# bzhangGo/zero

Measured on AMD Instinct MI355X. Metric: src+tgt tokens/sec training, Transformer-base d=512 L=6, higher is better.
Workload: dtype bf16; 1 GPU; Transformer-base (d=512, L=6+6, F=2048, h=8, V=32000) training step, B=64 x (src 64 + tgt 64) tokens per GPU, dropout 0.10, label_smooth 0.1, fwd+bwd+allreduce+Adam; model_name=transformer, parallelism=dp1, hip_graph=whole step

## Files before the change

### zero_amd/csrc/zk_attn_dev.h

```cpp
#pragma once
#include "zk_common.h"

typedef __bf16 bf16x8_t __attribute__((ext_vector_type(8)));
typedef float f32x4_t __attribute__((ext_vector_type(4)));

struct AttnArgs {
  const bf16_t* q; const bf16_t* k; const bf16_t* v;
  int ldq, ldk, ldv;
  long bsq, bsk, bsv;
  int kv_group;
  int B, nh, Lq, Lk, d;
  const float* kmask;
  int causal; int q_pos0;
  float scale; float mask_inf;
  const bf16_t* rpr_k; const bf16_t* rpr_v; int max_rel;
  uint32_t thr; float inv_keep; const uint64_t* seed; uint32_t sid;
  int ldmask;
  const int* pos_dev; int pos_flags;
  const float* gq; const float* gd; bf16_t* pb; bf16_t* dsb; int ldg; int nrp;
};

__device__ __forceinline__ void attn_apply_pos(AttnArgs& a) {
  if (a.pos_dev != nullptr) {
    const int t = *a.pos_dev;
// ... 133 lines not shown
}
__device__ __forceinline__ uint32_t half_of4(const uint4& v, int i) {
  const uint32_t w = (i >> 1) == 0 ? v.x : ((i >> 1) == 1 ? v.y : ((i >> 1) == 2 ? v.z : v.w));
  return (i & 1) ? (w >> 16) : (w & 0xffffu);
}
template <bool FRESH = false>
__device__ __forceinline__ void stage_trans(bf16_t* dst, const bf16_t* src, int ld, int row0, int nrows, int tid) {
  if (tid < 128) {
    const int dc = tid & 7, rq = tid >> 3;
    uint4 v[4];
#pragma unroll
    for (int u = 0; u < 4; ++u) {
      const int r = row0 + rq * 4 + u;
      v[u] = make_uint4(0u, 0u, 0u, 0u);
      if (r < nrows) v[u] = zk_ld16<FRESH>(src + (size_t)r * ld + dc * 8);
    }
#pragma unroll
    for (int i = 0; i < 8; ++i) {
      uint2 o;
      o.x = half_of4(v[0], i) | (half_of4(v[1], i) << 16);
      o.y = half_of4(v[2], i) | (half_of4(v[3], i) << 16);
      *reinterpret_cast<uint2*>(dst + (i * 8 + dc) * ALD + rq * 4) = o;
    }
  }
}
__device__ __forceinline__ int chan_of_phys(int q) { return (q & 7) * 8 + (q >> 3); }
struct DirectRegs { uint4 v[2]; };
template <bool FRESH = false>
__device__ __forceinline__ void load_direct(DirectRegs& R, const bf16_t* src, int ld, int row0, int nrows, int tid) {
#pragma unroll
  for (int it = 0; it < 2; ++it) {
    const int t = tid + it * 256;
    const int r = row0 + (t >> 3), c = (t & 7) * 8;
    const uint4 v = zk_ld16<FRESH>(src + (size_t)min(r, nrows - 1) * ld + c);
    R.v[it] = r < nrows ? v : make_uint4(0u, 0u, 0u, 0u);
  }
}
__device__ __forceinline__ void store_direct(bf16_t* dst, const DirectRegs& R, int tid) {
#pragma unroll
  for (int it = 0; it < 2; ++it) {
    const int t = tid + it * 256;
    *reinterpret_cast<uint4*>(dst + (t >> 3) * ALD + (t & 7) * 8) = R.v[it];
  }
}
struct TransRegs { uint4 v[4]; };
template <bool FRESH = false>
__device__ __forceinline__ void load_trans(TransRegs& R, const bf16_t* src, int ld, int row0, int nrows, int t128) {
  const int dc = t128 & 7, rq = t128 >> 3;
#pragma unroll
  for (int u = 0; u < 4; ++u) {
    const int r = row0 + rq * 4 + u;
    const uint4 v = zk_ld16<FRESH>(src + (size_t)min(r, nrows - 1) * ld + dc * 8);
    R.v[u] = r < nrows ? v : make_uint4(0u, 0u, 0u, 0u);
  }
}
__device__ __forceinline__ void store_trans(bf16_t* dst, const TransRegs& R, int t128) {
  const int dc = t128 & 7, rq = t128 >> 3;
#pragma unroll
  for (int i = 0; i < 8; ++i) {
    uint2 o;
    o.x = half_of4(R.v[0], i) | (half_of4(R.v[1], i) << 16);
    o.y = half_of4(R.v[2], i) | (half_of4(R.v[3], i) << 16);
    *reinterpret_cast<uint2*>(dst + (i * 8 + dc) * ALD + rq * 4) = o;
  }
}
__device__ __forceinline__ void store_tile_rows(const bf16_t* tile, bf16_t* dst, size_t ld, int nrows, int tid) {
#pragma unroll
  for (int it = 0; it < 2; ++it) {
    const int t = tid + it * 256;
    const int r = t >> 3, c = (t & 7) * 8;
    if (r < nrows) *reinterpret_cast<uint4*>(dst + (size_t)r * ld + c) = *reinterpret_cast<const uint4*>(tile + r * ALD + c);
  }
}

__device__ __forceinline__ float quad16_max(float v) {
  v = row16_max(v);
  return v;
}
__device__ __forceinline__ float quad16_sum(float v) {
  v = row16_sum(v);
  return v;
}

#define GLD 68
template <int NKT, bool RPR = false>
struct AttnFwdLds {
  static constexpr int BASE = (2 * TQ * ALD + TQ * (NKT * 64 + 8)) * 2;
  static constexpr int BYTES = BASE + (RPR ? 3 * TQ * ALD * 2 + TQ * GLD * 4 : 0);
};
template <int NKT, bool FRESH = false, bool RPR = false, int PRE = 0>
__device__ __forceinline__ void attn_fwd_tile(unsigned char* smem, const AttnArgs& a, bf16_t* __restrict__ out, int ldo,
                                              float* __restrict__ lse, int qt, int h, int b,
                                              const bf16_t* vt_pre = nullptr) {
  static_assert(PRE == 0 || PRE == 1 || (PRE == 3 && NKT == 1), "PRE = 3 is the single-tile self-attention");
  bf16_t* sQ = reinterpret_cast<bf16_t*>(smem);
  bf16_t* sK = sQ + TQ * ALD;
  bf16_t* sP = sK + TQ * ALD;
  constexpr int PLD = NKT * 64 + 8;
  [[maybe_unused]] bf16_t* sRk = reinterpret_cast<bf16_t*>(smem + AttnFwdLds<NKT, false>::BASE);
  [[maybe_unused]] bf16_t* sRvT = sRk + TQ * ALD;
  [[maybe_unused]] bf16_t* sPB = sRvT + TQ * ALD;
  [[maybe_unused]] float* sG = reinterpret_cast<float*>(sPB + TQ * ALD);
  [[maybe_unused]] const int nrel = 2 * a.max_rel + 1;
  const int tid = threadIdx.x, lane = tid & 63, w = tid >> 6;
  const int i0 = qt * TQ;
  const bf16_t* qb = a.q + (size_t)b * a.bsq + h * AD;
  const bf16_t* kb = a.k + (size_t)(b / a.kv_group) * a.bsk + h * AD;
  const bf16_t* vb = a.v + (size_t)(b / a.kv_group) * a.bsv + h * AD;
  const uint64_t seed = a.thr ? *a.seed : 0;

  DirectRegs rQ, rK;
  [[maybe_unused]] DirectRegs rRk;
  TransRegs rVt;
  if (PRE == 0) load_direct<FRESH>(rQ, qb, a.ldq, i0, a.Lq, tid);
  if (PRE != 3) {
    load_direct<FRESH>(rK, kb, a.ldk, 0, a.Lk, tid);
    if (tid < 128) load_trans<FRESH>(rVt, vb, a.ldv, 0, a.Lk, tid);
  }
  if (RPR) {
    load_direct(rRk, a.rpr_k, AD, 0, nrel, tid);
    if (tid >= 128) load_trans(rVt, a.rpr_v, AD, 0, nrel, tid - 128);
  }
  float kbias[NKT * 4];
#pragma unroll
  for (int t = 0; t < NKT * 4; ++t) {
    const int j = t * 16 + (lane & 15);
    kbias[t] = (a.kmask != nullptr && a.kmask[(size_t)(b / a.kv_group) * a.ldmask + min(j, a.Lk - 1)] == 0.f) ? -a.mask_inf : 0.f;
  }
  if (PRE == 0) store_direct(sQ, rQ, tid);
  if (PRE != 3) store_direct(sK, rK, tid);
  if (RPR) {
    store_direct(sRk, rRk, tid);
    if (tid >= 128) store_trans(sRvT, rVt, tid - 128);
  }
  f32x4_t S[NKT * 4];
#pragma unroll
  for (int kt = 0; kt < NKT; ++kt) {
    if (kt > 0) {
      __syncthreads();
      stage_direct<FRESH>(sK, kb, a.ldk, kt * 64, a.Lk, tid);
    }
    __syncthreads();
    const uint4 q0 = frag(sQ, w * 16, 0, lane), q1 = frag(sQ, w * 16, 1, lane);
#pragma unroll
    for (int nt = 0; nt < 4; ++nt) {
      f32x4_t acc = {0.f, 0.f, 0.f, 0.f};
      acc = mfma16(q0, frag(sK, nt * 16, 0, lane), acc);
      acc = mfma16(q1, frag(sK, nt * 16, 1, lane), acc);
      S[kt * 4 + nt] = acc;
    }
  }
  if (RPR) {
    const uint4 q0 = frag(sQ, w * 16, 0, lane), q1 = frag(sQ, w * 16, 1, lane);
#pragma unroll
    for (int nt = 0; nt < 4; ++nt) {
      f32x4_t acc = {0.f, 0.f, 0.f, 0.f};
      acc = mfma16(q0, frag(sRk, nt * 16, 0, lane), acc);
      acc = mfma16(q1, frag(sRk, nt * 16, 1, lane), acc);
#pragma unroll
      for (int r = 0; r < 4; ++r) sG[(w * 16 + (lane >> 4) * 4 + r) * GLD + nt * 16 + (lane & 15)] = acc[r];
    }
    __builtin_amdgcn_s_waitcnt(0xc07f);
    __builtin_amdgcn_wave_barrier();
  }
  const int rbase = i0 + w * 16 + (lane >> 4) * 4;
  float mx[4] = {-INFINITY, -INFINITY, -INFINITY, -INFINITY};
#pragma unroll
// ... 51 lines not shown
      const int il = w * 16 + (lane >> 4) * 4 + r;
      sP[il * PLD + j] = pb16;
      if (RPR) {
        const float pr = (rbase + r < a.Lq && j < a.Lk) ? bf2f(pb16) : 0.f;
        const int ri = rel_index(a.q_pos0 + rbase + r, j, a.max_rel);
        if (ri == 0) tlo[r] += pr;
        else if (ri == 2 * a.max_rel) thi[r] += pr;
        else sPB[il * ALD + ri] = f2bf(pr);
      }
    }
  }
  if (RPR) {
#pragma unroll
    for (int r = 0; r < 4; ++r) {
      const float s0 = row16_sum(tlo[r]), s1 = row16_sum(thi[r]);
      if ((lane & 15) == 0) {
        const int il = w * 16 + (lane >> 4) * 4 + r;
        sPB[il * ALD] = f2bf(s0);
        if (a.max_rel > 0) sPB[il * ALD + 2 * a.max_rel] = f2bf(s1);
      }
    }
  }
  if (a.pb != nullptr) {
    __builtin_amdgcn_s_waitcnt(0xc07f);
    __builtin_amdgcn_wave_barrier();
    rpr_bucket_rows(a, a.pb, b, h, i0, w, lane, [&](int row, int j) { return bf2f(sP[row * PLD + j]); });
  }
  f32x4_t O[4];
#pragma unroll
  for (int nb = 0; nb < 4; ++nb) O[nb] = (f32x4_t){0.f, 0.f, 0.f, 0.f};
#pragma unroll
  for (int kt = 0; kt < NKT; ++kt) {
    __syncthreads();
    if (kt == 0) { if (PRE != 3 && tid < 128) store_trans(sK, rVt, tid); }
    else stage_trans<FRESH>(sK, vb, a.ldv, kt * 64, a.Lk, tid);
    __syncthreads();
    const bf16_t* sVt = PRE == 3 ? vt_pre : sK;
#pragma unroll
    for (int kk = 0; kk < 2; ++kk) {
      const uint4 pa = *reinterpret_cast<const uint4*>(sP + (w * 16 + (lane & 15)) * PLD + kt * 64 + kk * 32 +
                                                       (lane >> 4) * 8);
#pragma unroll
      for (int nb = 0; nb < 4; ++nb) O[nb] = mfma16(pa, frag(sVt, nb * 16, kk, lane), O[nb]);
    }
  }
  if (RPR) {
    __builtin_amdgcn_s_waitcnt(0xc07f);
    __builtin_amdgcn_wave_barrier();
#pragma unroll
    for (int kk = 0; kk < 2; ++kk) {
      const uint4 pa = frag(sPB, w * 16, kk, lane);
#pragma unroll
      for (int nb = 0; nb < 4; ++nb) O[nb] = mfma16(pa, frag(sRvT, nb * 16, kk, lane), O[nb]);
    }
  }
#pragma unroll
  for (int nb = 0; nb < 4; ++nb) {
    const int c = chan_of_phys(nb * 16 + (lane & 15));
#pragma unroll
    for (int r = 0; r < 4; ++r) sQ[(w * 16 + (lane >> 4) * 4 + r) * ALD + c] = f2bf(O[nb][r]);
  }
  __syncthreads();
  store_tile_rows(sQ, out + ((size_t)b * a.Lq + i0) * ldo + h * AD, ldo, a.Lq - i0, tid);
}

#define ATTN_BWD64_LDS_BYTES (7 * TQ * ALD * 2 + TQ * 4)
#define ATTN_BWD64_RPR_LDS_BYTES (ATTN_BWD64_LDS_BYTES + 6 * TQ * ALD * 2 + 2 * TQ * GLD * 4)
struct AttnOProj { const bf16_t* dy; int lddy; const bf16_t* w; int ldw; int n; };
template <bool RPR = false, bool OPROJ = false>
__device__ __forceinline__ void attn_bwd_fused64_tile(unsigned char* smem, const AttnArgs& a, const bf16_t* __restrict__ o, int ldo,
                                                      const bf16_t* __restrict__ dout, int lddo,
                                                      const float* __restrict__ lse,
                                                      bf16_t* __restrict__ dq, int lddq,
                                                      bf16_t* __restrict__ dk, int lddk,
                                                      bf16_t* __restrict__ dv, int lddv, int h, int b,
                                                      float* __restrict__ rpr_part = nullptr,
                                                      const AttnOProj op = AttnOProj()) {
  bf16_t* sQ = reinterpret_cast<bf16_t*>(smem);
  bf16_t* sK = sQ + TQ * ALD;
  bf16_t* sV = sK + TQ * ALD;
  bf16_t* sdO = sV + TQ * ALD;
  bf16_t* sKt = sdO + TQ * ALD;
  bf16_t* sQt = sKt + TQ * ALD;
  bf16_t* sdOt = sQt + TQ * ALD;
  float* sL = reinterpret_cast<float*>(sdOt + TQ * ALD);
  [[maybe_unused]] bf16_t* sRk = reinterpret_cast<bf16_t*>(smem + ATTN_BWD64_LDS_BYTES);
  [[maybe_unused]] bf16_t* sRv = sRk + TQ * ALD;
  [[maybe_unused]] bf16_t* sRkT = sRv + TQ * ALD;
  [[maybe_unused]] bf16_t* sSB = sRkT + TQ * ALD;
  [[maybe_unused]] bf16_t* sSBt = sSB + TQ * ALD;
  [[maybe_unused]] bf16_t* sPBt = sSBt + TQ * ALD;
  [[maybe_unused]] float* sG = reinterpret_cast<float*>(sPBt + TQ * ALD);
  [[maybe_unused]] float* sGd = sG + TQ * GLD;
  const int tid = threadIdx.x, lane = tid & 63, w = tid >> 6;
  const bf16_t* qb = a.q + (size_t)b * a.bsq + h * AD;
  const bf16_t* kb = a.k + (size_t)b * a.bsk + h * AD;
  const bf16_t* vb = a.v + (size_t)b * a.bsv + h * AD;
  (void)o; (void)ldo;
  const bf16_t* dob = dout + (size_t)b * a.Lq * lddo + h * AD;
  const uint64_t seed = a.thr ? *a.seed : 0;

  ZK_AT(0);
  DirectRegs rQ, rdO, rK, rV;
  TransRegs t0, t1;
  load_direct(rQ, qb, a.ldq, 0, a.Lq, tid);
  if (!OPROJ) load_direct(rdO, dob, lddo, 0, a.Lq, tid);
  load_direct(rK, kb, a.ldk, 0, a.Lk, tid);
  load_direct(rV, vb, a.ldv, 0, a.Lk, tid);
  if (tid < 128) {
    load_trans(t0, kb, a.ldk, 0, a.Lk, tid);
  } else {
    load_trans(t0, qb, a.ldq, 0, a.Lq, tid - 128);
    if (!OPROJ) load_trans(t1, dob, lddo, 0, a.Lq, tid - 128);
  }
  [[maybe_unused]] f32x4_t dOa[4];
  [[maybe_unused]] DirectRegs wr[8];
  [[maybe_unused]] uint4 av[16];
  [[maybe_unused]] const bf16_t* wrow = OPROJ ? op.w + (size_t)h * AD * op.ldw : nullptr;
  [[maybe_unused]] const bf16_t* ap =
      OPROJ ? op.dy + ((size_t)b * a.Lq + min(w * 16 + (lane & 15), a.Lq - 1)) * op.lddy + (lane >> 4) * 8 : nullptr;
  auto oproj_issue = [&](int c0) {
    const int nsl = min(4, (op.n - c0) >> 7);
#pragma unroll
    for (int sl = 0; sl < 4; ++sl) {
      if (sl < nsl) {
        load_direct(wr[2 * sl], wrow + c0 + sl * 128, op.ldw, 0, AD, tid);
        load_direct(wr[2 * sl + 1], wrow + c0 + sl * 128 + 64, op.ldw, 0, AD, tid);
#pragma unroll
        for (int u = 0; u < 4; ++u) av[4 * sl + u] = zk_ld16<false>(ap + c0 + sl * 128 + u * 32);
      }
    }
  };
  if (OPROJ) {
#pragma unroll
    for (int nb = 0; nb < 4; ++nb) dOa[nb] = (f32x4_t){0.f, 0.f, 0.f, 0.f};
    oproj_issue(0);
  }
  const int dr = tid >> 2, dpart = tid & 3;
  const int drc = min(dr, a.Lq - 1);
  const float lse_r = lse[((size_t)b * a.nh + h) * a.Lq + drc];
  float kbias4[4];
#pragma unroll
  for (int nt = 0; nt < 4; ++nt) {
    const int j = nt * 16 + (lane & 15);
    kbias4[nt] = (a.kmask != nullptr && a.kmask[(size_t)b * a.ldmask + min(j, a.Lk - 1)] == 0.f) ? -a.mask_inf : 0.f;
  }
  if (OPROJ) {
    ZK_AT(1);
    for (int c0 = 0; c0 < op.n; c0 += 512) {
      const int nsl = min(4, (op.n - c0) >> 7);
      if (c0 > 0) oproj_issue(c0);
      else {
        store_direct(sQ, rQ, tid);
        store_direct(sK, rK, tid);
        store_direct(sV, rV, tid);
      }
#pragma unroll
      for (int sl = 0; sl < 4; ++sl) {
        if (sl < nsl) {
          bf16_t* w0 = sdO + (sl & 1) * 2 * TQ * ALD;
          bf16_t* w1 = w0 + TQ * ALD;
          store_direct(w0, wr[2 * sl], tid);
          store_direct(w1, wr[2 * sl + 1], tid);
          __syncthreads();
#pragma unroll
          for (int nb = 0; nb < 4; ++nb) {
            dOa[nb] = mfma16(av[4 * sl + 0], frag(w0, nb * 16, 0, lane), dOa[nb]);
            dOa[nb] = mfma16(av[4 * sl + 1], frag(w0, nb * 16, 1, lane), dOa[nb]);
            dOa[nb] = mfma16(av[4 * sl + 2], frag(w1, nb * 16, 0, lane), dOa[nb]);
            dOa[nb] = mfma16(av[4 * sl + 3], frag(w1, nb * 16, 1, lane), dOa[nb]);
          }
        }
      }
    }
    ZK_AT(2);
    __syncthreads();
  } else {
    store_direct(sQ, rQ, tid);
    store_direct(sdO, rdO, tid);
    store_direct(sK, rK, tid);
    store_direct(sV, rV, tid);
  }
  if (tid < 128) {
    store_trans(sKt, t0, tid);
  } else {
    store_trans(sQt, t0, tid - 128);
    if (!OPROJ) store_trans(sdOt, t1, tid - 128);
  }
  if (OPROJ) {
    const int r0 = w * 16 + (lane >> 4) * 4;
#pragma unroll
    for (int nb = 0; nb < 4; ++nb) {
      const int c = nb * 16 + (lane & 15);
      uint32_t hv[4];
#pragma unroll
      for (int r = 0; r < 4; ++r) {
        hv[r] = (r0 + r < a.Lq) ? (uint32_t)f2bf(dOa[nb][r]) : 0u;
        sdO[(r0 + r) * ALD + c] = (bf16_t)hv[r];
      }
      *reinterpret_cast<uint2*>(sdOt + ((c & 7) * 8 + (c >> 3)) * ALD + r0) = make_uint2(hv[0] | (hv[1] << 16), hv[2] | (hv[3] << 16));
    }
  }
  if (dpart == 0) sL[dr] = (dr < a.Lq) ? lse_r : 0.f;
  ZK_AT(3);
  if (RPR) {
    const int nrel = 2 * a.max_rel + 1;
    stage_direct(sRk, a.rpr_k, AD, 0, nrel, tid);
    stage_direct(sRv, a.rpr_v, AD, 0, nrel, tid);
    stage_trans(sRkT, a.rpr_k, AD, 0, nrel, tid);
    for (int e = tid; e < 3 * TQ * ALD / 8; e += 256)
      reinterpret_cast<uint4*>(sSB)[e] = make_uint4(0u, 0u, 0u, 0u);
  }
  __syncthreads();
  if (RPR) {
    const uint4 q0 = frag(sQ, w * 16, 0, lane), q1 = frag(sQ, w * 16, 1, lane);
    const uint4 g0 = frag(sdO, w * 16, 0, lane), g1 = frag(sdO, w * 16, 1, lane);
#pragma unroll
    for (int nt = 0; nt < 4; ++nt) {
      f32x4_t ga = {0.f, 0.f, 0.f, 0.f}, gb = {0.f, 0.f, 0.f, 0.f};
      ga = mfma16(q0, frag(sRk, nt * 16, 0, lane), ga);
      ga = mfma16(q1, frag(sRk, nt * 16, 1, lane), ga);
      gb = mfma16(g0, frag(sRv, nt * 16, 0, lane), gb);
      gb = mfma16(g1, frag(sRv, nt * 16, 1, lane), gb);
#pragma unroll
      for (int r = 0; r < 4; ++r) {
        sG[(w * 16 + (lane >> 4) * 4 + r) * GLD + nt * 16 + (lane & 15)] = ga[r];
        sGd[(w * 16 + (lane >> 4) * 4 + r) * GLD + nt * 16 + (lane & 15)] = gb[r];
      }
    }
    __builtin_amdgcn_s_waitcnt(0xc07f);
    __builtin_amdgcn_wave_barrier();
  }
  ZK_AT(4);
  const int rloc = w * 16 + (lane >> 4) * 4;
  float pv[4][4], dsv[4][4];
  {
    float pu[4][4], dpv[4][4], Di[4] = {0.f, 0.f, 0.f, 0.f};
    const uint4 q0 = frag(sQ, w * 16, 0, lane), q1 = frag(sQ, w * 16, 1, lane);
    const uint4 g0 = frag(sdO, w * 16, 0, lane), g1 = frag(sdO, w * 16, 1, lane);
#pragma unroll
    for (int nt = 0; nt < 4; ++nt) {
      f32x4_t sc4 = {0.f, 0.f, 0.f, 0.f}, dp = {0.f, 0.f, 0.f, 0.f};
// ... 9 lines not shown
        const int i = rloc + r;
        const bool live = kvalid && i < a.Lq;
        float raw = sc4[r], dpr = dp[r];
        if (a.gq != nullptr && live) { raw += rpr_gather(a, a.gq, b, h, i, j); dpr += rpr_gather(a, a.gd, b, h, i, j); }
        if (RPR && live) {
          const int ri = rel_index(a.q_pos0 + i, j, a.max_rel);
          raw += sG[i * GLD + ri];
          dpr += sGd[i * GLD + ri];
        }
        float sc = raw * a.scale + kbias;
        if (a.causal && j > a.q_pos0 + i) sc -= a.mask_inf;
        const float p = live ? __expf(sc - sL[i]) : 0.f;
        float ms = 1.f;
        if (a.thr) {
          const uint64_t idx = (((uint64_t)b * a.nh + h) * a.Lq + i) * a.Lk + j;
          ms = zk_drop_scale(seed, a.sid, idx, a.thr, a.inv_keep);
        }
        pv[nt][r] = p * ms;
        pu[nt][r] = p;
        dpv[nt][r] = dpr * ms;
        Di[r] += p * dpr * ms;
      }
    }
#pragma unroll
    for (int r = 0; r < 4; ++r) {
      Di[r] = row16_sum(Di[r]);
    }
#pragma unroll
    for (int nt = 0; nt < 4; ++nt)
#pragma unroll
      for (int r = 0; r < 4; ++r) dsv[nt][r] = pu[nt][r] * (dpv[nt][r] - Di[r]) * a.scale;
  }
  ZK_AT(5);
  __syncthreads();
  ZK_AT(6);
  bf16_t* sdS = sQ;
  bf16_t* sPt = sK;
  bf16_t* sdSt = sV;
#pragma unroll
  for (int nt = 0; nt < 4; ++nt) {
    const int j = nt * 16 + (lane & 15);
    uint2 pp, dd;
    pp.x = (uint32_t)f2bf(pv[nt][0]) | ((uint32_t)f2bf(pv[nt][1]) << 16);
    pp.y = (uint32_t)f2bf(pv[nt][2]) | ((uint32_t)f2bf(pv[nt][3]) << 16);
    dd.x = (uint32_t)f2bf(dsv[nt][0]) | ((uint32_t)f2bf(dsv[nt][1]) << 16);
    dd.y = (uint32_t)f2bf(dsv[nt][2]) | ((uint32_t)f2bf(dsv[nt][3]) << 16);
    *reinterpret_cast<uint2*>(sPt + j * ALD + rloc) = pp;
    *reinterpret_cast<uint2*>(sdSt + j * ALD + rloc) = dd;
#pragma unroll
    for (int r = 0; r < 4; ++r) sdS[(rloc + r) * ALD + j] = f2bf(dsv[nt][r]);
  }
  __syncthreads();
  if (RPR) {
    rpr_bucket_wave(a, 2 * a.max_rel + 1, 0, w, lane, [&](int row, int j) { return bf2f(sdS[row * ALD + j]); },
                    [&](int row, int r, float v) { const bf16_t x = f2bf(v); sSB[row * ALD + r] = x; sSBt[r * ALD + row] = x; });
    rpr_bucket_wave(a, 2 * a.max_rel + 1, 0, w, lane, [&](int row, int j) { return bf2f(sPt[j * ALD + row]); },
                    [&](int row, int r, float v) { sPBt[r * ALD + row] = f2bf(v); });
    __syncthreads();
  }
  if (a.dsb != nullptr) {
    rpr_bucket_rows(a, a.dsb, b, h, 0, w, lane, [&](int row, int j) { return bf2f(sdS[row * ALD + j]); });
    rpr_bucket_rows(a, a.pb, b, h, 0, w, lane, [&](int row, int j) { return bf2f(sPt[j * ALD + row]); });
  }
  ZK_AT(7);
  f32x4_t dQ[4], dK[4], dV[4];
#pragma unroll
  for (int nb = 0; nb < 4; ++nb) {
    dQ[nb] = (f32x4_t){0.f, 0.f, 0.f, 0.f};
    dK[nb] = (f32x4_t){0.f, 0.f, 0.f, 0.f};
    dV[nb] = (f32x4_t){0.f, 0.f, 0.f, 0.f};
  }
#pragma unroll
  for (int kk = 0; kk < 2; ++kk) {
    const uint4 da = frag(sdS, w * 16, kk, lane);
    const uint4 pa = frag(sPt, w * 16, kk, lane);
    const uint4 dt = frag(sdSt, w * 16, kk, lane);
#pragma unroll
    for (int nb = 0; nb < 4; ++nb) {
      dQ[nb] = mfma16(da, frag(sKt, nb * 16, kk, lane), dQ[nb]);
      dV[nb] = mfma16(pa, frag(sdOt, nb * 16, kk, lane), dV[nb]);
      dK[nb] = mfma16(dt, frag(sQt, nb * 16, kk, lane), dK[nb]);
    }
  }
  ZK_AT(8);
  if (RPR) {
    f32x4_t tk[4], tv[4];
#pragma unroll
    for (int nb = 0; nb < 4; ++nb) { tk[nb] = (f32x4_t){0.f, 0.f, 0.f, 0.f}; tv[nb] = (f32x4_t){0.f, 0.f, 0.f, 0.f}; }
#pragma unroll
    for (int kk = 0; kk < 2; ++kk) {
      const uint4 sb = frag(sSB, w * 16, kk, lane);
      const uint4 st = frag(sSBt, w * 16, kk, lane);
      const uint4 pt = frag(sPBt, w * 16, kk, lane);
#pragma unroll
      for (int nb = 0; nb < 4; ++nb) {
        dQ[nb] = mfma16(sb, frag(sRkT, nb * 16, kk, lane), dQ[nb]);
        tk[nb] = mfma16(st, frag(sQt, nb * 16, kk, lane), tk[nb]);
        tv[nb] = mfma16(pt, frag(sdOt, nb * 16, kk, lane), tv[nb]);
      }
    }
    float* pk = rpr_part + ((size_t)b * a.nh + h) * 2 * TQ * AD;
#pragma unroll
    for (int nb = 0; nb < 4; ++nb) {
      const int c = chan_of_phys(nb * 16 + (lane & 15));
#pragma unroll
      for (int r = 0; r < 4; ++r) {
        sG[(rloc + r) * GLD + c] = tk[nb][r];
        sGd[(rloc + r) * GLD + c] = tv[nb][r];
      }
    }
    __builtin_amdgcn_s_waitcnt(0xc07f);
    __builtin_amdgcn_wave_barrier();
    const int nrel = 2 * a.max_rel + 1;
#pragma unroll
    for (int it = 0; it < 4; ++it) {
      const int e = it * 64 + lane, rr = w * 16 + (e >> 4), c4 = (e & 15) * 4;
      if (rr < nrel) {
        *reinterpret_cast<float4*>(pk + rr * AD + c4) = *reinterpret_cast<const float4*>(sG + rr * GLD + c4);
        *reinterpret_cast<float4*>(pk + TQ * AD + rr * AD + c4) = *reinterpret_cast<const float4*>(sGd + rr * GLD + c4);
      }
    }
  }
  __syncthreads();
  bf16_t* oQ = sKt; bf16_t* oK = sQt; bf16_t* oV = sdOt;
#pragma unroll
  for (int nb = 0; nb < 4; ++nb) {
    const int c = chan_of_phys(nb * 16 + (lane & 15));
#pragma unroll
    for (int r = 0; r < 4; ++r) {
      const int i = rloc + r;
      oQ[i * ALD + c] = f2bf(dQ[nb][r]);
      oK[i * ALD + c] = f2bf(dK[nb][r]);
      oV[i * ALD + c] = f2bf(dV[nb][r]);
    }
  }
  __syncthreads();
  ZK_AT(9);
  store_tile_rows(oQ, dq + (size_t)b * a.Lq * lddq + h * AD, lddq, a.Lq, tid);
  store_tile_rows(oK, dk + (size_t)b * a.Lk * lddk + h * AD, lddk, a.Lk, tid);
  store_tile_rows(oV, dv + (size_t)b * a.Lk * lddv + h * AD, lddv, a.Lk, tid);
  ZK_AT(10);
}

#define ATTN_BWD64_RPR2_LDS_BYTES (8 * TQ * ALD * 2 + TQ * 4)
__device__ __forceinline__ void attn_bwd_rpr64_tile(unsigned char* smem, const AttnArgs& a,
                                                    const bf16_t* __restrict__ dout, int lddo,
                                                    const float* __restrict__ lse,
                                                    bf16_t* __restrict__ dq, int lddq,
                                                    bf16_t* __restrict__ dk, int lddk,
                                                    bf16_t* __restrict__ dv, int lddv, int h, int b,
                                                    float* __restrict__ rpr_part) {
  constexpr int TB = TQ * ALD;
  bf16_t* T0 = reinterpret_cast<bf16_t*>(smem);
  bf16_t* T1 = T0 + TB; bf16_t* T2 = T1 + TB; bf16_t* T3 = T2 + TB;
  bf16_t* T4 = T3 + TB; bf16_t* T5 = T4 + TB; bf16_t* T6 = T5 + TB; bf16_t* T7 = T6 + TB;
  float* sG = reinterpret_cast<float*>(T6);
  float* sL = reinterpret_cast<float*>(T7 + TB);
  static_assert(TQ * GLD * 4 <= 2 * TQ * ALD * 2, "G must fit two tiles");
  static_assert(2 * TQ * GLD * 4 <= 4 * TQ * ALD * 2, "the two table partials must fit four tiles");
  const int tid = threadIdx.x, lane = tid & 63, w = tid >> 6;
  const bf16_t* qb = a.q + (size_t)b * a.bsq + h * AD;
  const bf16_t* kb = a.k + (size_t)b * a.bsk + h * AD;
  const bf16_t* vb = a.v + (size_t)b * a.bsv + h * AD;
  const bf16_t* dob = dout + (size_t)b * a.Lq * lddo + h * AD;
  const uint64_t seed = a.thr ? *a.seed : 0;
  const int nrel = 2 * a.max_rel + 1;

  ZK_AT(0);
  DirectRegs rQ, rdO, rK, rV, rRk, rRv;
  TransRegs t0, t1;
  load_direct(rQ, qb, a.ldq, 0, a.Lq, tid);
  load_direct(rdO, dob, lddo, 0, a.Lq, tid);
  load_direct(rK, kb, a.ldk, 0, a.Lk, tid);
  load_direct(rV, vb, a.ldv, 0, a.Lk, tid);
  load_direct(rRk, a.rpr_k, AD, 0, nrel, tid);
  load_direct(rRv, a.rpr_v, AD, 0, nrel, tid);
  if (tid < 128) {
    load_trans(t0, kb, a.ldk, 0, a.Lk, tid);
    load_trans(t1, a.rpr_k, AD, 0, nrel, tid);
  } else {
    load_trans(t0, qb, a.ldq, 0, a.Lq, tid - 128);
    load_trans(t1, dob, lddo, 0, a.Lq, tid - 128);
  }
  const int dr = tid >> 2, dpart = tid & 3;
  const float lse_r = lse[((size_t)b * a.nh + h) * a.Lq + min(dr, a.Lq - 1)];
  float kbias4[4];
#pragma unroll
  for (int nt = 0; nt < 4; ++nt) {
    const int j = nt * 16 + (lane & 15);
    kbias4[nt] = (a.kmask != nullptr && a.kmask[(size_t)b * a.ldmask + min(j, a.Lk - 1)] == 0.f) ? -a.mask_inf : 0.f;
  }
  store_direct(T0, rQ, tid);
  store_direct(T3, rdO, tid);
  store_direct(T1, rK, tid);
  store_direct(T2, rV, tid);
  store_direct(T4, rRk, tid);
  store_direct(T5, rRv, tid);
  if (dpart == 0) sL[dr] = (dr < a.Lq) ? lse_r : 0.f;
  ZK_AT(3);
  __syncthreads();
  ZK_AT(4);

  const int rloc = w * 16 + (lane >> 4) * 4;
  float pv[4][4], dsv[4][4];
  {
    float pu[4][4], Di[4] = {0.f, 0.f, 0.f, 0.f};
    uint32_t kept = 0;
    const uint4 q0 = frag(T0, w * 16, 0, lane), q1 = frag(T0, w * 16, 1, lane);
    const uint4 g0 = frag(T3, w * 16, 0, lane), g1 = frag(T3, w * 16, 1, lane);
#pragma unroll
    for (int nt = 0; nt < 4; ++nt) {
      f32x4_t ga = {0.f, 0.f, 0.f, 0.f};
      ga = mfma16(q0, frag(T4, nt * 16, 0, lane), ga);
      ga = mfma16(q1, frag(T4, nt * 16, 1, lane), ga);
#pragma unroll
      for (int r = 0; r < 4; ++r) sG[(rloc + r) * GLD + nt * 16 + (lane & 15)] = ga[r];
    }
    __builtin_amdgcn_s_waitcnt(0xc07f);
    __builtin_amdgcn_wave_barrier();
#pragma unroll
    for (int nt = 0; nt < 4; ++nt) {
      f32x4_t sc4 = {0.f, 0.f, 0.f, 0.f};
      sc4 = mfma16(q0, frag(T1, nt * 16, 0, lane), sc4);
      sc4 = mfma16(q1, frag(T1, nt * 16, 1, lane), sc4);
      const int j = nt * 16 + (lane & 15);
      const bool kvalid = j < a.Lk;
      const float kbias = kvalid ? kbias4[nt] : 0.f;
#pragma unroll
      for (int r = 0; r < 4; ++r) {
        const int i = rloc + r;
        const bool live = kvalid && i < a.Lq;
// ... 39 lines not shown
        if (kvalid && i < a.Lq) dpr += sG[i * GLD + rel_index(a.q_pos0 + i, j, a.max_rel)];
        const float ms = ((kept >> (nt * 4 + r)) & 1u) ? (a.thr ? a.inv_keep : 1.f) : 0.f;
        dpv[nt][r] = dpr * ms;
        Di[r] += pu[nt][r] * dpr * ms;
      }
    }
#pragma unroll
    for (int r = 0; r < 4; ++r) Di[r] = row16_sum(Di[r]);
#pragma unroll
    for (int nt = 0; nt < 4; ++nt)
#pragma unroll
      for (int r = 0; r < 4; ++r) dsv[nt][r] = pu[nt][r] * (dpv[nt][r] - Di[r]) * a.scale;
  }
  ZK_AT(5);
  __syncthreads();
  ZK_AT(6);
  bf16_t* sdS = T0; bf16_t* sPt = T1; bf16_t* sdSt = T2;
  bf16_t* sKt = T3; bf16_t* sRkT = T4; bf16_t* sQt = T6; bf16_t* sdOt = T7;
  uint2 ppk[4], ddk[4];
#pragma unroll
  for (int nt = 0; nt < 4; ++nt) {
    const int j = nt * 16 + (lane & 15);
    uint2 pp, dd;
    pp.x = (uint32_t)f2bf(pv[nt][0]) | ((uint32_t)f2bf(pv[nt][1]) << 16);
    pp.y = (uint32_t)f2bf(pv[nt][2]) | ((uint32_t)f2bf(pv[nt][3]) << 16);
    dd.x = (uint32_t)f2bf(dsv[nt][0]) | ((uint32_t)f2bf(dsv[nt][1]) << 16);
    dd.y = (uint32_t)f2bf(dsv[nt][2]) | ((uint32_t)f2bf(dsv[nt][3]) << 16);
    ppk[nt] = pp; ddk[nt] = dd;
    *reinterpret_cast<uint2*>(sPt + j * ALD + rloc) = pp;
    *reinterpret_cast<uint2*>(sdSt + j * ALD + rloc) = dd;
#pragma unroll
    for (int r = 0; r < 4; ++r) sdS[(rloc + r) * ALD + j] = (bf16_t)((r & 1) ? ((r & 2 ? dd.y : dd.x) >> 16) : ((r & 2 ? dd.y : dd.x) & 0xffffu));
  }
  if (tid < 128) {
    store_trans(sKt, t0, tid);
    store_trans(sRkT, t1, tid);
  } else {
    store_trans(sQt, t0, tid - 128);
    store_trans(sdOt, t1, tid - 128);
  }
  __syncthreads();
  ZK_AT(7);
  f32x4_t dQ[4], dK[4], dV[4];
#pragma unroll
  for (int nb = 0; nb < 4; ++nb) {
    dQ[nb] = (f32x4_t){0.f, 0.f, 0.f, 0.f};
    dK[nb] = (f32x4_t){0.f, 0.f, 0.f, 0.f};
    dV[nb] = (f32x4_t){0.f, 0.f, 0.f, 0.f};
  }
#pragma unroll
  for (int kk = 0; kk < 2; ++kk) {
    const uint4 da = frag(sdS, w * 16, kk, lane);
    const uint4 pa = frag(sPt, w * 16, kk, lane);
    const uint4 dt = frag(sdSt, w * 16, kk, lane);
#pragma unroll
    for (int nb = 0; nb < 4; ++nb) {
      dQ[nb] = mfma16(da, frag(sKt, nb * 16, kk, lane), dQ[nb]);
      dV[nb] = mfma16(pa, frag(sdOt, nb * 16, kk, lane), dV[nb]);
      dK[nb] = mfma16(dt, frag(sQt, nb * 16, kk, lane), dK[nb]);
    }
  }
  ZK_AT(8);
  __syncthreads();
  bf16_t* sSB = T2; bf16_t* sSBt = T3; bf16_t* sPBt = T5;
  {
    const uint4 z = make_uint4(0u, 0u, 0u, 0u);
#pragma unroll
    for (int it = 0; it < 2; ++it) {
      const int e = it * 64 + lane;
      *reinterpret_cast<uint4*>(sSB + (w * 16 + (e >> 3)) * ALD + (e & 7) * 8) = z;
      *reinterpret_cast<uint4*>(sSBt + (e >> 1) * ALD + w * 16 + (e & 1) * 8) = z;
      *reinterpret_cast<uint4*>(sPBt + (e >> 1) * ALD + w * 16 + (e & 1) * 8) = z;
    }
// ... 85 lines not shown
```

Before: 2.005 million src+tgt tokens/s.

## Use LDS transpose reads in fused attention backward, drop transposed tile copies

The fused 64-token attention backward now reads K, Q, dO and dS directly from their row-major LDS tiles with ds_read_tr16_b64 transpose loads. This removes the separately staged transposed copies (Kt, Qt, dOt, RkT, dS), their global loads and LDS stores, and one barrier, and it shrinks the RPR LDS footprint. It also hoists the kmask and lse loads ahead of the tile loads, moves the zero-masking of out-of-range rows from the load into the store, and templatises the O-projection chunk loop on a compile-time slice count. The cost is reliance on the gfx950 transpose-read instruction and a changed channel ordering (chan_of_phys removed in the backward path), which must stay consistent with the rest of the kernel.

```diff
diff --git a/zero_amd/csrc/zk_attn_dev.h b/zero_amd/csrc/zk_attn_dev.h
--- a/zero_amd/csrc/zk_attn_dev.h
+++ b/zero_amd/csrc/zk_attn_dev.h
@@ -189,11 +189,24 @@
   for (int it = 0; it < 2; ++it) {
     const int t = tid + it * 256;
     const int r = row0 + (t >> 3), c = (t & 7) * 8;
-    const uint4 v = zk_ld16<FRESH>(src + (size_t)min(r, nrows - 1) * ld + c);
-    R.v[it] = r < nrows ? v : make_uint4(0u, 0u, 0u, 0u);
-  }
-}
-__device__ __forceinline__ void store_direct(bf16_t* dst, const DirectRegs& R, int tid) {
+    R.v[it] = zk_ld16<FRESH>(src + (size_t)min(r, nrows - 1) * ld + c);
+  }
+}
+__device__ __forceinline__ void load_direct64(DirectRegs& R, const bf16_t* src, int ld, int tid) {
+#pragma unroll
+  for (int it = 0; it < 2; ++it) {
+    const int t = tid + it * 256;
+    R.v[it] = zk_ld16<false>(src + (size_t)(t >> 3) * ld + (t & 7) * 8);
+  }
+}
+__device__ __forceinline__ void store_direct(bf16_t* dst, const DirectRegs& R, int tid, int nlive) {
+#pragma unroll
+  for (int it = 0; it < 2; ++it) {
+    const int t = tid + it * 256;
+    *reinterpret_cast<uint4*>(dst + (t >> 3) * ALD + (t & 7) * 8) = (t >> 3) < nlive ? R.v[it] : make_uint4(0u, 0u, 0u, 0u);
+  }
+}
+__device__ __forceinline__ void store_direct64(bf16_t* dst, const DirectRegs& R, int tid) {
 #pragma unroll
   for (int it = 0; it < 2; ++it) {
     const int t = tid + it * 256;
@@ -207,19 +220,44 @@
 #pragma unroll
   for (int u = 0; u < 4; ++u) {
     const int r = row0 + rq * 4 + u;
-    const uint4 v = zk_ld16<FRESH>(src + (size_t)min(r, nrows - 1) * ld + dc * 8);
-    R.v[u] = r < nrows ? v : make_uint4(0u, 0u, 0u, 0u);
-  }
-}
-__device__ __forceinline__ void store_trans(bf16_t* dst, const TransRegs& R, int t128) {
+    R.v[u] = zk_ld16<FRESH>(src + (size_t)min(r, nrows - 1) * ld + dc * 8);
+  }
+}
+__device__ __forceinline__ void store_trans(bf16_t* dst, const TransRegs& R, int t128, int nlive) {
   const int dc = t128 & 7, rq = t128 >> 3;
+  uint4 v[4];
+#pragma unroll
+  for (int u = 0; u < 4; ++u) v[u] = rq * 4 + u < nlive ? R.v[u] : make_uint4(0u, 0u, 0u, 0u);
 #pragma unroll
   for (int i = 0; i < 8; ++i) {
     uint2 o;
-    o.x = half_of4(R.v[0], i) | (half_of4(R.v[1], i) << 16);
-    o.y = half_of4(R.v[2], i) | (half_of4(R.v[3], i) << 16);
+    o.x = half_of4(v[0], i) | (half_of4(v[1], i) << 16);
+    o.y = half_of4(v[2], i) | (half_of4(v[3], i) << 16);
     *reinterpret_cast<uint2*>(dst + (i * 8 + dc) * ALD + rq * 4) = o;
   }
+}
+typedef short attn_v4s_t __attribute__((ext_vector_type(4)));
+__device__ __forceinline__ uint4 frag_tr(const bf16_t* t, int c0, int kk, int lane) {
+  const int p = lane & 15;
+  const bf16_t* a = t + (kk * 32 + (lane >> 4) * 8 + (p >> 2)) * ALD + c0 + (p & 3) * 4;
+  const attn_v4s_t lo = __builtin_amdgcn_ds_read_tr16_b64_v4i16((__attribute__((address_space(3))) attn_v4s_t*)a);
+  const attn_v4s_t hi = __builtin_amdgcn_ds_read_tr16_b64_v4i16((__attribute__((address_space(3))) attn_v4s_t*)(a + 4 * ALD));
+  typedef short attn_v8s_t __attribute__((ext_vector_type(8)));
+  const attn_v8s_t both = __builtin_shufflevector(lo, hi, 0, 1, 2, 3, 4, 5, 6, 7);
+  return __builtin_bit_cast(uint4, both);
+}
+template <int N>
+__device__ __forceinline__ void kmask_load(float (&m)[N], const AttnArgs& a, int bk, int lane) {
+  const bool has = a.kmask != nullptr;
+  const float* row = has ? a.kmask + (size_t)bk * a.ldmask : reinterpret_cast<const float*>(a.q);
+#pragma unroll
+  for (int t = 0; t < N; ++t) m[t] = row[has ? min(t * 16 + (lane & 15), a.Lk - 1) : 0];
+}
+template <int N>
+__device__ __forceinline__ void kmask_bias(float (&m)[N], const AttnArgs& a) {
+  const bool has = a.kmask != nullptr;
+#pragma unroll
+  for (int t = 0; t < N; ++t) m[t] = (has && m[t] == 0.f) ? -a.mask_inf : 0.f;
 }
 __device__ __forceinline__ void store_tile_rows(const bf16_t* tile, bf16_t* dst, size_t ld, int nrows, int tid) {
 #pragma unroll
@@ -269,6 +307,8 @@
   DirectRegs rQ, rK;
   [[maybe_unused]] DirectRegs rRk;
   TransRegs rVt;
+  float kbias[NKT * 4];
+  kmask_load(kbias, a, b / a.kv_group, lane);
   if (PRE == 0) load_direct<FRESH>(rQ, qb, a.ldq, i0, a.Lq, tid);
   if (PRE != 3) {
     load_direct<FRESH>(rK, kb, a.ldk, 0, a.Lk, tid);
@@ -278,18 +318,13 @@
     load_direct(rRk, a.rpr_k, AD, 0, nrel, tid);
     if (tid >= 128) load_trans(rVt, a.rpr_v, AD, 0, nrel, tid - 128);
   }
-  float kbias[NKT * 4];
-#pragma unroll
-  for (int t = 0; t < NKT * 4; ++t) {
-    const int j = t * 16 + (lane & 15);
-    kbias[t] = (a.kmask != nullptr && a.kmask[(size_t)(b / a.kv_group) * a.ldmask + min(j, a.Lk - 1)] == 0.f) ? -a.mask_inf : 0.f;
-  }
-  if (PRE == 0) store_direct(sQ, rQ, tid);
-  if (PRE != 3) store_direct(sK, rK, tid);
+  if (PRE == 0) store_direct(sQ, rQ, tid, a.Lq - i0);
+  if (PRE != 3) store_direct(sK, rK, tid, a.Lk);
   if (RPR) {
-    store_direct(sRk, rRk, tid);
-    if (tid >= 128) store_trans(sRvT, rVt, tid - 128);
-  }
+    store_direct(sRk, rRk, tid, nrel);
+    if (tid >= 128) store_trans(sRvT, rVt, tid - 128, nrel);
+  }
+  kmask_bias(kbias, a);
   f32x4_t S[NKT * 4];
 #pragma unroll
   for (int kt = 0; kt < NKT; ++kt) {
@@ -407,7 +442,7 @@
 #pragma unroll
   for (int kt = 0; kt < NKT; ++kt) {
     __syncthreads();
-    if (kt == 0) { if (PRE != 3 && tid < 128) store_trans(sK, rVt, tid); }
+    if (kt == 0) { if (PRE != 3 && tid < 128) store_trans(sK, rVt, tid, a.Lk); }
     else stage_trans<FRESH>(sK, vb, a.ldv, kt * 64, a.Lk, tid);
     __syncthreads();
     const bf16_t* sVt = PRE == 3 ? vt_pre : sK;
@@ -440,8 +475,9 @@
 }
 
 #define ATTN_BWD64_LDS_BYTES (7 * TQ * ALD * 2 + TQ * 4)
-#define ATTN_BWD64_RPR_LDS_BYTES (ATTN_BWD64_LDS_BYTES + 6 * TQ * ALD * 2 + 2 * TQ * GLD * 4)
+#define ATTN_BWD64_RPR_LDS_BYTES (ATTN_BWD64_LDS_BYTES + 5 * TQ * ALD * 2 + 2 * TQ * GLD * 4)
 struct AttnOProj { const bf16_t* dy; int lddy; const bf16_t* w; int ldw; int n; };
+template <int V> struct zk_int_c { static constexpr int value = V; };
 template <bool RPR = false, bool OPROJ = false>
 __device__ __forceinline__ void attn_bwd_fused64_tile(unsigned char* smem, const AttnArgs& a, const bf16_t* __restrict__ o, int ldo,
                                                       const bf16_t* __restrict__ dout, int lddo,
@@ -455,14 +491,13 @@
   bf16_t* sK = sQ + TQ * ALD;
   bf16_t* sV = sK + TQ * ALD;
   bf16_t* sdO = sV + TQ * ALD;
-  bf16_t* sKt = sdO + TQ * ALD;
-  bf16_t* sQt = sKt + TQ * ALD;
-  bf16_t* sdOt = sQt + TQ * ALD;
-  float* sL = reinterpret_cast<float*>(sdOt + TQ * ALD);
+  bf16_t* sdSt = sdO + TQ * ALD;
+  bf16_t* sPt = sdSt + TQ * ALD;
+  bf16_t* sT6 = sPt + TQ * ALD;
+  float* sL = reinterpret_cast<float*>(sT6 + TQ * ALD);
   [[maybe_unused]] bf16_t* sRk = reinterpret_cast<bf16_t*>(smem + ATTN_BWD64_LDS_BYTES);
   [[maybe_unused]] bf16_t* sRv = sRk + TQ * ALD;
-  [[maybe_unused]] bf16_t* sRkT = sRv + TQ * ALD;
-  [[maybe_unused]] bf16_t* sSB = sRkT + TQ * ALD;
+  [[maybe_unused]] bf16_t* sSB = sRv + TQ * ALD;
   [[maybe_unused]] bf16_t* sSBt = sSB + TQ * ALD;
   [[maybe_unused]] bf16_t* sPBt = sSBt + TQ * ALD;
   [[maybe_unused]] float* sG = reinterpret_cast<float*>(sPBt + TQ * ALD);
@@ -476,113 +511,89 @@
   const uint64_t seed = a.thr ? *a.seed : 0;
 
   ZK_AT(0);
+  const int dr = tid >> 2, dpart = tid & 3;
+  const float lse_r = lse[((size_t)b * a.nh + h) * a.Lq + min(dr, a.Lq - 1)];
+  float kbias4[4];
+  kmask_load(kbias4, a, b, lane);
   DirectRegs rQ, rdO, rK, rV;
-  TransRegs t0, t1;
   load_direct(rQ, qb, a.ldq, 0, a.Lq, tid);
   if (!OPROJ) load_direct(rdO, dob, lddo, 0, a.Lq, tid);
   load_direct(rK, kb, a.ldk, 0, a.Lk, tid);
   load_direct(rV, vb, a.ldv, 0, a.Lk, tid);
-  if (tid < 128) {
-    load_trans(t0, kb, a.ldk, 0, a.Lk, tid);
-  } else {
-    load_trans(t0, qb, a.ldq, 0, a.Lq, tid - 128);
-    if (!OPROJ) load_trans(t1, dob, lddo, 0, a.Lq, tid - 128);
-  }
   [[maybe_unused]] f32x4_t dOa[4];
-  [[maybe_unused]] DirectRegs wr[8];
-  [[maybe_unused]] uint4 av[16];
   [[maybe_unused]] const bf16_t* wrow = OPROJ ? op.w + (size_t)h * AD * op.ldw : nullptr;
   [[maybe_unused]] const bf16_t* ap =
       OPROJ ? op.dy + ((size_t)b * a.Lq + min(w * 16 + (lane & 15), a.Lq - 1)) * op.lddy + (lane >> 4) * 8 : nullptr;
-  auto oproj_issue = [&](int c0) {
-    const int nsl = min(4, (op.n - c0) >> 7);
-#pragma unroll
-    for (int sl = 0; sl < 4; ++sl) {
-      if (sl < nsl) {
-        load_direct(wr[2 * sl], wrow + c0 + sl * 128, op.ldw, 0, AD, tid);
-        load_direct(wr[2 * sl + 1], wrow + c0 + sl * 128 + 64, op.ldw, 0, AD, tid);
-#pragma unroll
-        for (int u = 0; u < 4; ++u) av[4 * sl + u] = zk_ld16<false>(ap + c0 + sl * 128 + u * 32);
-      }
+  auto oproj_chunk = [&](int c0, auto nsl_c, auto first_c) {
+    constexpr int NSL = decltype(nsl_c)::value;
+    DirectRegs wr[2 * NSL];
+    uint4 av[4 * NSL];
+#pragma unroll
+    for (int sl = 0; sl < NSL; ++sl) {
+      load_direct64(wr[2 * sl], wrow + c0 + sl * 128, op.ldw, tid);
+      load_direct64(wr[2 * sl + 1], wrow + c0 + sl * 128 + 64, op.ldw, tid);
+#pragma unroll
+      for (int u = 0; u < 4; ++u) av[4 * sl + u] = zk_ld16<false>(ap + c0 + sl * 128 + u * 32);
+    }
+    if (decltype(first_c)::value) {
+      ZK_AT(1);
+      store_direct(sQ, rQ, tid, a.Lq);
+      store_direct(sK, rK, tid, a.Lk);
+      store_direct(sV, rV, tid, a.Lk);
+    }
+#pragma unroll
+    for (int sl = 0; sl < NSL; ++sl) {
+      bf16_t* w0 = sdO + (sl & 1) * 2 * TQ * ALD;
+      bf16_t* w1 = w0 + TQ * ALD;
+      store_direct64(w0, wr[2 * sl], tid);
+      store_direct64(w1, wr[2 * sl + 1], tid);
+      __syncthreads();
+#pragma unroll
+      for (int nb = 0; nb < 4; ++nb) {
+        dOa[nb] = mfma16(av[4 * sl + 0], frag(w0, nb * 16, 0, lane), dOa[nb]);
+        dOa[nb] = mfma16(av[4 * sl + 1], frag(w0, nb * 16, 1, lane), dOa[nb]);
+        dOa[nb] = mfma16(av[4 * sl + 2], frag(w1, nb * 16, 0, lane), dOa[nb]);
+        dOa[nb] = mfma16(av[4 * sl + 3], frag(w1, nb * 16, 1, lane), dOa[nb]);
+      }
+    }
+  };
+  auto oproj_dispatch = [&](int c0, auto first_c) {
+    switch (min(4, (op.n - c0) >> 7)) {
+      case 4: oproj_chunk(c0, zk_int_c<4>(), first_c); break;
+      case 3: oproj_chunk(c0, zk_int_c<3>(), first_c); break;
+      case 2: oproj_chunk(c0, zk_int_c<2>(), first_c); break;
+      default: oproj_chunk(c0, zk_int_c<1>(), first_c); break;
     }
   };
   if (OPROJ) {
 #pragma unroll
     for (int nb = 0; nb < 4; ++nb) dOa[nb] = (f32x4_t){0.f, 0.f, 0.f, 0.f};
-    oproj_issue(0);
-  }
-  const int dr = tid >> 2, dpart = tid & 3;
-  const int drc = min(dr, a.Lq - 1);
-  const float lse_r = lse[((size_t)b * a.nh + h) * a.Lq + drc];
-  float kbias4[4];
-#pragma unroll
-  for (int nt = 0; nt < 4; ++nt) {
-    const int j = nt * 16 + (lane & 15);
-    kbias4[nt] = (a.kmask != nullptr && a.kmask[(size_t)b * a.ldmask + min(j, a.Lk - 1)] == 0.f) ? -a.mask_inf : 0.f;
-  }
-  if (OPROJ) {
-    ZK_AT(1);
-    for (int c0 = 0; c0 < op.n; c0 += 512) {
-      const int nsl = min(4, (op.n - c0) >> 7);
-      if (c0 > 0) oproj_issue(c0);
-      else {
-        store_direct(sQ, rQ, tid);
-        store_direct(sK, rK, tid);
-        store_direct(sV, rV, tid);
-      }
-#pragma unroll
-      for (int sl = 0; sl < 4; ++sl) {
-        if (sl < nsl) {
-          bf16_t* w0 = sdO + (sl & 1) * 2 * TQ * ALD;
-          bf16_t* w1 = w0 + TQ * ALD;
-          store_direct(w0, wr[2 * sl], tid);
-          store_direct(w1, wr[2 * sl + 1], tid);
-          __syncthreads();
-#pragma unroll
-          for (int nb = 0; nb < 4; ++nb) {
-            dOa[nb] = mfma16(av[4 * sl + 0], frag(w0, nb * 16, 0, lane), dOa[nb]);
-            dOa[nb] = mfma16(av[4 * sl + 1], frag(w0, nb * 16, 1, lane), dOa[nb]);
-            dOa[nb] = mfma16(av[4 * sl + 2], frag(w1, nb * 16, 0, lane), dOa[nb]);
-            dOa[nb] = mfma16(av[4 * sl + 3], frag(w1, nb * 16, 1, lane), dOa[nb]);
-          }
-        }
-      }
-    }
+    oproj_dispatch(0, zk_int_c<1>());
+    for (int c0 = 512; c0 < op.n; c0 += 512) oproj_dispatch(c0, zk_int_c<0>());
     ZK_AT(2);
     __syncthreads();
   } else {
-    store_direct(sQ, rQ, tid);
-    store_direct(sdO, rdO, tid);
-    store_direct(sK, rK, tid);
-    store_direct(sV, rV, tid);
-  }
-  if (tid < 128) {
-    store_trans(sKt, t0, tid);
-  } else {
-    store_trans(sQt, t0, tid - 128);
-    if (!OPROJ) store_trans(sdOt, t1, tid - 128);
+    store_direct(sQ, rQ, tid, a.Lq);
+    store_direct(sdO, rdO, tid, a.Lq);
+    store_direct(sK, rK, tid, a.Lk);
+    store_direct(sV, rV, tid, a.Lk);
   }
   if (OPROJ) {
     const int r0 = w * 16 + (lane >> 4) * 4;
 #pragma unroll
     for (int nb = 0; nb < 4; ++nb) {
       const int c = nb * 16 + (lane & 15);
-      uint32_t hv[4];
-#pragma unroll
-      for (int r = 0; r < 4; ++r) {
-        hv[r] = (r0 + r < a.Lq) ? (uint32_t)f2bf(dOa[nb][r]) : 0u;
-        sdO[(r0 + r) * ALD + c] = (bf16_t)hv[r];
-      }
-      *reinterpret_cast<uint2*>(sdOt + ((c & 7) * 8 + (c >> 3)) * ALD + r0) = make_uint2(hv[0] | (hv[1] << 16), hv[2] | (hv[3] << 16));
+#pragma unroll
+      for (int r = 0; r < 4; ++r) sdO[(r0 + r) * ALD + c] = (r0 + r < a.Lq) ? f2bf(dOa[nb][r]) : (bf16_t)0;
     }
   }
   if (dpart == 0) sL[dr] = (dr < a.Lq) ? lse_r : 0.f;
+  kmask_bias(kbias4, a);
   ZK_AT(3);
   if (RPR) {
     const int nrel = 2 * a.max_rel + 1;
     stage_direct(sRk, a.rpr_k, AD, 0, nrel, tid);
     stage_direct(sRv, a.rpr_v, AD, 0, nrel, tid);
-    stage_trans(sRkT, a.rpr_k, AD, 0, nrel, tid);
     for (int e = tid; e < 3 * TQ * ALD / 8; e += 256)
       reinterpret_cast<uint4*>(sSB)[e] = make_uint4(0u, 0u, 0u, 0u);
   }
@@ -658,11 +669,6 @@
       for (int r = 0; r < 4; ++r) dsv[nt][r] = pu[nt][r] * (dpv[nt][r] - Di[r]) * a.scale;
   }
   ZK_AT(5);
-  __syncthreads();
-  ZK_AT(6);
-  bf16_t* sdS = sQ;
-  bf16_t* sPt = sK;
-  bf16_t* sdSt = sV;
 #pragma unroll
   for (int nt = 0; nt < 4; ++nt) {
     const int j = nt * 16 + (lane & 15);
@@ -673,19 +679,17 @@
     dd.y = (uint32_t)f2bf(dsv[nt][2]) | ((uint32_t)f2bf(dsv[nt][3]) << 16);
     *reinterpret_cast<uint2*>(sPt + j * ALD + rloc) = pp;
     *reinterpret_cast<uint2*>(sdSt + j * ALD + rloc) = dd;
-#pragma unroll
-    for (int r = 0; r < 4; ++r) sdS[(rloc + r) * ALD + j] = f2bf(dsv[nt][r]);
   }
   __syncthreads();
   if (RPR) {
-    rpr_bucket_wave(a, 2 * a.max_rel + 1, 0, w, lane, [&](int row, int j) { return bf2f(sdS[row * ALD + j]); },
+    rpr_bucket_wave(a, 2 * a.max_rel + 1, 0, w, lane, [&](int row, int j) { return bf2f(sdSt[j * ALD + row]); },
                     [&](int row, int r, float v) { const bf16_t x = f2bf(v); sSB[row * ALD + r] = x; sSBt[r * ALD + row] = x; });
     rpr_bucket_wave(a, 2 * a.max_rel + 1, 0, w, lane, [&](int row, int j) { return bf2f(sPt[j * ALD + row]); },
                     [&](int row, int r, float v) { sPBt[r * ALD + row] = f2bf(v); });
     __syncthreads();
   }
   if (a.dsb != nullptr) {
-    rpr_bucket_rows(a, a.dsb, b, h, 0, w, lane, [&](int row, int j) { return bf2f(sdS[row * ALD + j]); });
+    rpr_bucket_rows(a, a.dsb, b, h, 0, w, lane, [&](int row, int j) { return bf2f(sdSt[j * ALD + row]); });
     rpr_bucket_rows(a, a.pb, b, h, 0, w, lane, [&](int row, int j) { return bf2f(sPt[j * ALD + row]); });
   }
   ZK_AT(7);
@@ -698,14 +702,14 @@
   }
 #pragma unroll
   for (int kk = 0; kk < 2; ++kk) {
-    const uint4 da = frag(sdS, w * 16, kk, lane);
+    const uint4 da = frag_tr(sdSt, w * 16, kk, lane);
     const uint4 pa = frag(sPt, w * 16, kk, lane);
     const uint4 dt = frag(sdSt, w * 16, kk, lane);
 #pragma unroll
     for (int nb = 0; nb < 4; ++nb) {
-      dQ[nb] = mfma16(da, frag(sKt, nb * 16, kk, lane), dQ[nb]);
-      dV[nb] = mfma16(pa, frag(sdOt, nb * 16, kk, lane), dV[nb]);
-      dK[nb] = mfma16(dt, frag(sQt, nb * 16, kk, lane), dK[nb]);
+      dQ[nb] = mfma16(da, frag_tr(sK, nb * 16, kk, lane), dQ[nb]);
+      dV[nb] = mfma16(pa, frag_tr(sdO, nb * 16, kk, lane), dV[nb]);
+      dK[nb] = mfma16(dt, frag_tr(sQ, nb * 16, kk, lane), dK[nb]);
     }
   }
   ZK_AT(8);
@@ -720,15 +724,15 @@
       const uint4 pt = frag(sPBt, w * 16, kk, lane);
 #pragma unroll
       for (int nb = 0; nb < 4; ++nb) {
-        dQ[nb] = mfma16(sb, frag(sRkT, nb * 16, kk, lane), dQ[nb]);
-        tk[nb] = mfma16(st, frag(sQt, nb * 16, kk, lane), tk[nb]);
-        tv[nb] = mfma16(pt, frag(sdOt, nb * 16, kk, lane), tv[nb]);
+        dQ[nb] = mfma16(sb, frag_tr(sRk, nb * 16, kk, lane), dQ[nb]);
+        tk[nb] = mfma16(st, frag_tr(sQ, nb * 16, kk, lane), tk[nb]);
+        tv[nb] = mfma16(pt, frag_tr(sdO, nb * 16, kk, lane), tv[nb]);
       }
     }
     float* pk = rpr_part + ((size_t)b * a.nh + h) * 2 * TQ * AD;
 #pragma unroll
     for (int nb = 0; nb < 4; ++nb) {
-      const int c = chan_of_phys(nb * 16 + (lane & 15));
+      const int c = nb * 16 + (lane & 15);
 #pragma unroll
       for (int r = 0; r < 4; ++r) {
         sG[(rloc + r) * GLD + c] = tk[nb][r];
@@ -748,10 +752,10 @@
     }
   }
   __syncthreads();
-  bf16_t* oQ = sKt; bf16_t* oK = sQt; bf16_t* oV = sdOt;
+  bf16_t* oQ = sdSt; bf16_t* oK = sPt; bf16_t* oV = sT6;
 #pragma unroll
   for (int nb = 0; nb < 4; ++nb) {
-    const int c = chan_of_phys(nb * 16 + (lane & 15));
+    const int c = nb * 16 + (lane & 15);
 #pragma unroll
     for (int r = 0; r < 4; ++r) {
       const int i = rloc + r;
@@ -793,6 +797,10 @@
   const int nrel = 2 * a.max_rel + 1;
 
   ZK_AT(0);
+  const int dr = tid >> 2, dpart = tid & 3;
+  const float lse_r = lse[((size_t)b * a.nh + h) * a.Lq + min(dr, a.Lq - 1)];
+  float kbias4[4];
+  kmask_load(kbias4, a, b, lane);
   DirectRegs rQ, rdO, rK, rV, rRk, rRv;
   TransRegs t0, t1;
   load_direct(rQ, qb, a.ldq, 0, a.Lq, tid);
@@ -801,28 +809,17 @@
   load_direct(rV, vb, a.ldv, 0, a.Lk, tid);
   load_direct(rRk, a.rpr_k, AD, 0, nrel, tid);
   load_direct(rRv, a.rpr_v, AD, 0, nrel, tid);
-  if (tid < 128) {
-    load_trans(t0, kb, a.ldk, 0, a.Lk, tid);
-    load_trans(t1, a.rpr_k, AD, 0, nrel, tid);
-  } else {
-    load_trans(t0, qb, a.ldq, 0, a.Lq, tid - 128);
-    load_trans(t1, dob, lddo, 0, a.Lq, tid - 128);
-  }
-  const int dr = tid >> 2, dpart = tid & 3;
-  const float lse_r = lse[((size_t)b * a.nh + h) * a.Lq + min(dr, a.Lq - 1)];
-  float kbias4[4];
-#pragma unroll
-  for (int nt = 0; nt < 4; ++nt) {
-    const int j = nt * 16 + (lane & 15);
-    kbias4[nt] = (a.kmask != nullptr && a.kmask[(size_t)b * a.ldmask + min(j, a.Lk - 1)] == 0.f) ? -a.mask_inf : 0.f;
-  }
-  store_direct(T0, rQ, tid);
-  store_direct(T3, rdO, tid);
-  store_direct(T1, rK, tid);
-  store_direct(T2, rV, tid);
-  store_direct(T4, rRk, tid);
-  store_direct(T5, rRv, tid);
+  const bool lo128 = tid < 128;
+  load_trans(t0, lo128 ? kb : qb, lo128 ? a.ldk : a.ldq, 0, lo128 ? a.Lk : a.Lq, tid & 127);
+  load_trans(t1, lo128 ? a.rpr_k : dob, lo128 ? AD : lddo, 0, lo128 ? nrel : a.Lq, tid & 127);
+  store_direct(T0, rQ, tid, a.Lq);
+  store_direct(T3, rdO, tid, a.Lq);
+  store_direct(T1, rK, tid, a.Lk);
+  store_direct(T2, rV, tid, a.Lk);
+  store_direct(T4, rRk, tid, nrel);
+  store_direct(T5, rRv, tid, nrel);
   if (dpart == 0) sL[dr] = (dr < a.Lq) ? lse_r : 0.f;
+  kmask_bias(kbias4, a);
   ZK_AT(3);
   __syncthreads();
   ZK_AT(4);
@@ -928,13 +925,8 @@
 #pragma unroll
     for (int r = 0; r < 4; ++r) sdS[(rloc + r) * ALD + j] = (bf16_t)((r & 1) ? ((r & 2 ? dd.y : dd.x) >> 16) : ((r & 2 ? dd.y : dd.x) & 0xffffu));
   }
-  if (tid < 128) {
-    store_trans(sKt, t0, tid);
-    store_trans(sRkT, t1, tid);
-  } else {
-    store_trans(sQt, t0, tid - 128);
-    store_trans(sdOt, t1, tid - 128);
-  }
+  store_trans(lo128 ? sKt : sQt, t0, tid & 127, lo128 ? a.Lk : a.Lq);
+  store_trans(lo128 ? sRkT : sdOt, t1, tid & 127, lo128 ? nrel : a.Lq);
   __syncthreads();
   ZK_AT(7);
   f32x4_t dQ[4], dK[4], dV[4];
```

Measured after the change: 2.038 million src+tgt tokens/s (median of 6 runs). 1.6% higher.
